# toandaominh1997/EfficientDet.Pytorch

Hardware: AMD Instinct MI355X
Metric: images/sec EfficientDet-D0 512px fwd+bwd (higher is better)
Workload: dtype f32_hf16x3_bwd_bf16x3

## Files before the change

efficientdet/pytorch_amd/_lib.py:

```python
import ctypes as C
import os

import torch

HERE = os.path.dirname(os.path.abspath(__file__))
LIB_PATH = os.environ.get('EFFDET_HIP_LIB') or os.path.join(os.path.dirname(os.path.abspath(__file__)), 'libeffdet_hip.so')
MAX_SEG = 5
MAX_CONV_SEG = 10
ABI_VERSION = 11
F32, BF16, F32_BF16X3, F32_SPLIT = 0, 1, 2, 3
F32_HSPLIT = 4
ACT_NONE, ACT_RELU, ACT_SWISH, ACT_SIGMOID = 0, 1, 2, 3
RES_NONE, RES_ADD, RES_RELU_MASK, RES_SWISH_GRAD = 0, 1, 2, 3
TUNE_IGEMM_BIG, TUNE_IGEMM_BIG_MIN_M, TUNE_SPLIT_PERS, TUNE_IGEMM_KORD, TUNE_SPLIT_KORD = 0, 1, 2, 3, 4

_ERR = {-1: 'EFFDET_EINVAL', -2: 'EFFDET_ELAUNCH', -3: 'EFFDET_EUNSUPPORTED'}


class Seg(C.Structure):
    _fields_ = [('H', C.c_int), ('W', C.c_int), ('Ho', C.c_int), ('Wo', C.c_int),
                ('in_off', C.c_longlong), ('in_bstride', C.c_longlong),
                ('out_off', C.c_longlong), ('out_bstride', C.c_longlong)]


# ... 195 lines not shown
}
SYMBOLS = list(SIGNATURES)
ADDED_SIGNATURES = {
    'effdet_soft_nms_workspace_bytes': 'q:iqi',
    'effdet_soft_nms': 'i:pppffifiiippppqiqs',
}
EMA_SIGNATURES = {
    'effdet_clip_adamw_step_ema': 'i:ppppppppiippffffffifipps',
    'effdet_clip_adamw_step_gated_ema': 'i:pppppppppiippfffffffippps',
    'effdet_ema_swap': 'i:pppppiis',
}
PLAN_SIGNATURES = {
    'effdet_dwconv_plan_info': 'i:iiiiiiiiiiiiip',
}
LIVE_SIGNATURES = {
    'effdet_live_tiles_counts': 'q:iipppp',
    'effdet_live_tiles': 'i:piiiippppps',
    'effdet_conv2d_live': 'i:ppis',
    'effdet_conv2d_wgrad_live': 'i:ppqps',
}
NEEDED_SIGNATURES = {
    'effdet_positive_pixel_map': 'i:ppiqiippps',
    'effdet_live_tiles_from_map': 'i:piippppps',
    'effdet_conv2d_needed': 'i:ppis',
}
BOX_LOSS_SIGNATURES = {
    'effdet_box_loss_fwd': 'i:ppppppqiqiiifs',
    'effdet_box_loss_fwd_grad': 'i:ppppppqpiiiqiiifs',
    'effdet_box_loss_bwd_reg': 'i:ppppppiiiqiifs',
}
LOSS_OPTS_SIGNATURES = {
    'effdet_loss_opts_workspace_bytes': 'q:iqii',
    'effdet_loss_opts_fwd': 'i:ppppppqiqiips',
    'effdet_loss_opts_fwd_grad': 'i:ppppppqpiiiqiips',
    'effdet_loss_opts_bwd_cls': 'i:pppppiiiqiips',
    'effdet_loss_opts_bwd_reg': 'i:ppppppiiiqips',
}
ATSS_SIGNATURES = {
    'effdet_loss_atss_workspace_bytes': 'q:iqiip',
    'effdet_loss_atss_fwd': 'i:ppppppqiqiipps',
    'effdet_loss_atss_fwd_grad': 'i:ppppppqpiiiqiipps',
}
CONV_PLAN_SIGNATURES = {
    'effdet_conv2d_plan_info': 'i:pp',
}
WBF_SIGNATURES = {
    'effdet_wbf_workspace_bytes': 'q:iii',
    'effdet_wbf': 'i:ppqs',
}
MOSAIC_SIGNATURES = {
    'effdet_mosaic_compose': 'i:ppppiiips',
    'effdet_mosaic_boxes': 'i:ppiipiffpips',
}
CONV_FORMS = ('plain', 'bf16x3', 'split', 'hsplit', 'skinny')
LIVE_RADII = 6
DW_PLAN_FWD, DW_PLAN_DGRAD, DW_PLAN_WGRAD, DW_PLAN_BWD, DW_PLAN_EXPAND_FWD = 0, 1, 2, 3, 4
DW_INFO = ('cq', 'tpi', 'ppt', 'nbuf', 'groups', 'nslab', 'direct')


def lib():
    global _lib
    if _lib is None:
        if not os.path.exists(LIB_PATH):
            raise RuntimeError(
                'libeffdet_hip.so is missing (%s). Build it with `python -m efficientdet.pytorch_amd.build` '
                '(or __graft_entry__.build()). There is no CPU fallback for this path.' % LIB_PATH)
        cand = C.CDLL(LIB_PATH)
        got = int(cand.effdet_abi_version()) if hasattr(cand, 'effdet_abi_version') else 0
        if got != ABI_VERSION:
            raise RuntimeError('%s has ABI generation %d, this binding needs %d: rebuild it (`python -m efficientdet.pytorch_amd.build`)'
                               % (LIB_PATH, got, ABI_VERSION))
        _lib = cand
        for name, sig in list(SIGNATURES.items()) + list(ADDED_SIGNATURES.items()) + list(EMA_SIGNATURES.items()) + \
                list(PLAN_SIGNATURES.items()) + list(LIVE_SIGNATURES.items()) + list(BOX_LOSS_SIGNATURES.items()) + \
                list(LOSS_OPTS_SIGNATURES.items()) + list(ATSS_SIGNATURES.items()) + list(CONV_PLAN_SIGNATURES.items()) + \
                list(WBF_SIGNATURES.items()) + list(NEEDED_SIGNATURES.items()) + list(MOSAIC_SIGNATURES.items()):
            f = getattr(_lib, name, None)
            if f is not None:
                f.restype, f.argtypes = _CTYPE[sig[0]], [_CTYPE[c] for c in sig[2:]]
    return _lib


def require(*names):
    L = lib()
    missing = [n for n in names if not hasattr(L, n)]
    if missing:
        raise RuntimeError('%s does not export %s: it predates this binding, rebuild it (`python -m efficientdet.pytorch_amd.build`)'
                           % (LIB_PATH, ', '.join(missing)))
    return L


def check(status, what):
    if status != 0:
        raise RuntimeError('%s failed: %s (%d)' % (what, _ERR.get(status, 'unknown'), status))


_raw_stream = getattr(torch._C, '_cuda_getCurrentRawStream', None)


def stream_ptr():
    if _raw_stream is not None:
        return _raw_stream(torch.cuda.current_device())
    return torch.cuda.current_stream().cuda_stream


def ptr(t):
    return None if t is None else t.data_ptr()


def dtype_code(t):
    if t == torch.float32:
        return F32
    if t == torch.bfloat16:
        return BF16
    raise TypeError('unsupported storage dtype %s' % t)
```

efficientdet/pytorch_amd/csrc/conv_wgrad.hip:

```cpp
#include "common.h"
#include "../../../include/effdet_live_tiles.h"
#include <stdlib.h>

#ifndef EFFDET_WGRAD_TR_WAVES
#define EFFDET_WGRAD_TR_WAVES 8
#endif

namespace {

struct WSeg {
  int H, W, Ho, Wo, M, split_start;
  long long in_off, in_bs, out_off, out_bs;
  unsigned x_bytes, dz_bytes;
  int step0;
};
struct WgradK {
  const void* x; const void* dz; float* dw; float* dbias; float* slab;
  float* dbp;
  int Cin, Cout, KW, stride, pad_t, pad_l;
  int ldx, lddz;
  int B;
  int Kc, cpt;
  int K;
  int mchunk;
  int nseg, ntiles, jtiles, vec_a;
  const unsigned char* live32;
  WSeg seg[EFFDET_MAX_SEG];
};

template <typename T> struct WMma;
template <> struct WMma<bf16_t> {
  static __device__ __forceinline__ void run(const uint4& a, const uint4& b, f32x4& c) {
    c = __builtin_amdgcn_mfma_f32_16x16x32_bf16(__builtin_bit_cast(bf16x8, a), __builtin_bit_cast(bf16x8, b), c, 0, 0, 0);
  }
  static __device__ __forceinline__ uint4 ones() { return make_uint4(0x3f803f80u, 0x3f803f80u, 0x3f803f80u, 0x3f803f80u); }
};
template <> struct WMma<float> {
  static __device__ __forceinline__ void run(const uint4& a, const uint4& b, f32x4& c) {
    c = __builtin_amdgcn_mfma_f32_16x16x4f32(__uint_as_float(a.x), __uint_as_float(b.x), c, 0, 0, 0);
    c = __builtin_amdgcn_mfma_f32_16x16x4f32(__uint_as_float(a.y), __uint_as_float(b.y), c, 0, 0, 0);
    c = __builtin_amdgcn_mfma_f32_16x16x4f32(__uint_as_float(a.z), __uint_as_float(b.z), c, 0, 0, 0);
    c = __builtin_amdgcn_mfma_f32_16x16x4f32(__uint_as_float(a.w), __uint_as_float(b.w), c, 0, 0, 0);
  }
  static __device__ __forceinline__ uint4 ones() { return make_uint4(0x3f800000u, 0x3f800000u, 0x3f800000u, 0x3f800000u); }
};

__device__ __forceinline__ int swz(int row) { return ((row >> 1) & 7) ^ ((row >> 4) & 7); }

template <typename T> struct Transpose;
template <> struct Transpose<float> {
  static __device__ __forceinline__ void run(const uint4 (&in)[4], uint4 (&out)[4]) {
    out[0] = make_uint4(in[0].x, in[1].x, in[2].x, in[3].x);
    out[1] = make_uint4(in[0].y, in[1].y, in[2].y, in[3].y);
    out[2] = make_uint4(in[0].z, in[1].z, in[2].z, in[3].z);
// ... 294 lines not shown
  }
  const bool want_bias = (p.dbp != nullptr) && (jt == 0) && (wj0 == 0);
  const uint4 ones = WMma<bf16_t>::ones();
  const int l15 = lane & 15, lq = lane >> 4;
  float* slab = p.slab + (long long)split * p.Cout * p.K;

  if (nsteps > 0) {
    stage(0);
    for (int kt = 0; kt < nsteps; ++kt) {
      const unsigned cur = (unsigned)(kt & 1) * BUFB;
      dma_wait_all();
      __syncthreads();
      if (kt + 1 < nsteps) stage((kt & 1) ^ 1);
#pragma unroll
      for (int ks = 0; ks < 2; ++ks) {
        uint4 af[4], bf[JT];
#pragma unroll
        for (int a = 0; a < 4; ++a) af[a] = frag(a_addr[a] + cur + (unsigned)ks * 8192u);
#pragma unroll
        for (int b = 0; b < JT; ++b) bf[b] = frag(b_addr[b] + cur + (unsigned)ks * 8192u);
#pragma unroll
        for (int a = 0; a < 4; ++a)
#pragma unroll
          for (int b = 0; b < JT; ++b) WMma<bf16_t>::run(af[a], bf[b], acc[a][b]);
        if (want_bias) {
#pragma unroll
          for (int a = 0; a < 4; ++a) WMma<bf16_t>::run(af[a], ones, bsum[a]);
        }
      }
    }
#pragma unroll
    for (int a = 0; a < 4; ++a) {
#pragma unroll
      for (int rr = 0; rr < 4; ++rr) {
        const int n = nt * 128 + wn0 + a * 16 + lq * 4 + rr;
        if (n >= p.Cout) continue;
#pragma unroll
        for (int b = 0; b < JT; ++b) {
          const int j = jt * 128 + wj0 + b * 16 + l15;
          if (j < p.K) slab[(long long)n * p.K + j] = acc[a][b][rr];
        }
        if (want_bias && l15 == 0) p.dbp[(long long)split * p.Cout + n] = bsum[a][rr];
      }
    }
  } else {
    for (int i = tid; i < 128 * 128; i += NW * 64) {
      const int n = nt * 128 + i / 128, j = jt * 128 + (i & 127);
      if (n < p.Cout && j < p.K) slab[(long long)n * p.K + j] = 0.f;
    }
    if (p.dbp && jt == 0 && tid < 128 && nt * 128 + tid < p.Cout) p.dbp[(long long)split * p.Cout + nt * 128 + tid] = 0.f;
  }
}

template <int ALLR, int LIVE = 0>
__global__ __launch_bounds__(512) void conv_wgrad_split_kernel(const WgradK p) {
  constexpr unsigned OPB = 16384, BUFB = 2 * OPB, RG = 4096;
  extern __shared__ __attribute__((aligned(16))) uint4 smem[];
  const int tid = threadIdx.x, lane = tid & 63;
  const int wave = __builtin_amdgcn_readfirstlane(tid >> 6);
  const int wn = wave >> 2, wj = wave & 3;
  const int logical = xcd_remap(blockIdx.x, gridDim.x);
  const int nt = logical % p.ntiles, jt = (logical / p.ntiles) % p.jtiles, split = logical / (p.ntiles * p.jtiles);
  int si = 0;
#pragma unroll
  for (int s = 1; s < EFFDET_MAX_SEG; ++s)
    if (s < p.nseg && split >= p.seg[s].split_start) si = s;
  const WSeg sg = p.seg[si];
  const int m_begin = (split - sg.split_start) * p.mchunk;
  const int m_end = min(sg.M, m_begin + p.mchunk);
  const int nsteps = (m_end - m_begin + 31) / 32;

  const bool stage_x = wave >= 4;
  const int rgi = wave & 3;
  const int Wr = sg.Wo < 8 ? sg.Wo : 8, RP = 8 / Wr;
  const int r = lane >> 3, g = (lane & 7) ^ (((r >> 1) & 3) << 1);
  const int dho = r / Wr, dwo = r - dho * Wr;
  int off_s[4]; unsigned flg[4];
#pragma unroll
  for (int hf = 0; hf < 4; ++hf) {
    if (!stage_x) {
      const int n = nt * 256 + hf * 64 + g * 8;
      off_s[hf] = (r * p.lddz + n) * 2;
      flg[hf] = (n + 8 > p.lddz) ? 1u : 0u;
    } else {
      const int jq = jt * 32 + hf * 8 + g;
      const bool jok = jq < p.Kc;
      const int tap = jok ? jq / p.cpt : 0, cc = jok ? jq - tap * p.cpt : 0;
      const int kh = tap / p.KW, kw = tap - kh * p.KW;
      const int dkh = kh - p.pad_t, dkw = kw - p.pad_l;
      off_s[hf] = ((dkh * sg.W + dkw + r) * p.ldx + cc * 8) * 2;
      flg[hf] = (jok ? 0u : 1u) | ((dkh < 0 && dho == 0) ? 2u : 0u) | ((dkh > 0 && dho == RP - 1) ? 4u : 0u) |
                ((dkw < 0 && dwo == 0) ? 8u : 0u) | ((dkw > 0 && dwo == Wr - 1) ? 16u : 0u);
    }
  }
  const u32x4_t srd = stage_x ? make_srd_raw((const bf16_t*)p.x + sg.in_off, sg.x_bytes)
                              : make_srd_raw((const bf16_t*)p.dz + sg.out_off, sg.dz_bytes);
  const u32x4_t srd_u = u32x4_t{(unsigned)__builtin_amdgcn_readfirstlane((int)srd[0]), (unsigned)__builtin_amdgcn_readfirstlane((int)srd[1]),
                                (unsigned)__builtin_amdgcn_readfirstlane((int)srd[2]), (unsigned)__builtin_amdgcn_readfirstlane((int)srd[3])};
  const unsigned s_bs = (unsigned)((stage_x ? sg.in_bs : sg.out_bs) * 2), s_ld = (unsigned)((stage_x ? p.ldx : p.lddz) * 2);
  const unsigned lds0 = lds_addr(smem);
  const unsigned dst0 = lds0 + (stage_x ? OPB : 0u) + (unsigned)rgi * RG;

  const int HoWo = sg.Ho * sg.Wo;
  int cm = m_begin + 8 * rgi;
  int cb = cm / HoWo, crem = cm - cb * HoWo;
  int cho = crem / sg.Wo, cwo = crem - cho * sg.Wo;
  auto seek = [&](int step) {
    cm = m_begin + 32 * step + 8 * rgi;
    cb = cm / HoWo; crem = cm - cb * HoWo;
    cho = crem / sg.Wo; cwo = crem - cho * sg.Wo;
  };
  const unsigned char* const lv = LIVE ? p.live32 + sg.step0 + m_begin / 32 : nullptr;
  int lwin = -1; unsigned long long lmask = 0ull;
  auto next_live = [&](int s) -> int {
    while (s < nsteps) {
      if ((s >> 6) != lwin) {
        lwin = s >> 6;
        const int i = lwin * 64 + lane;
        lmask = __ballot(i < nsteps && lv[i] != 0);
      }
      const unsigned long long rest = lmask >> (s & 63);
      if (rest) return s + __builtin_ctzll(rest);
      s = (s | 63) + 1;
    }
    return nsteps;
  };
  auto stage = [&](int buf) {
    const bool all_out = cm >= m_end;
    const unsigned cmask = 1u | (cho == 0 ? 2u : 0u) | (cho == sg.Ho - RP ? 4u : 0u) | (cwo == 0 ? 8u : 0u) | (cwo == sg.Wo - Wr ? 16u : 0u);
    const unsigned base = (unsigned)cb * s_bs + (unsigned)(cho * sg.Wo + cwo) * s_ld;
    const unsigned dst = dst0 + (unsigned)buf * BUFB;
#pragma unroll
    for (int hf = 0; hf < 4; ++hf)
      dma16_async(srd_u, dst + (unsigned)hf * 1024u, (all_out || (flg[hf] & cmask)) ? EFFDET_OOB : base + (unsigned)off_s[hf]);
    cm += 32; cwo += 32;
    while (cwo >= sg.Wo) { cwo -= sg.Wo; if (++cho == sg.Ho) { cho = 0; ++cb; } }
  };

  const int s16 = lane & 15, q = lane >> 4, jrow = s16 >> 2;
  const unsigned lane_base = (unsigned)(q >> 1) * RG + (unsigned)((q & 1) * 4 + jrow) * 128u + (unsigned)(s16 & 3) * 8u;
  const int xr = (q & 1) * 2 + (jrow >> 1);
  unsigned a_addr[2][4], b_addr[4];
#pragma unroll
  for (int gi = 0; gi < 2; ++gi)
#pragma unroll
    for (int k = 0; k < 4; ++k) a_addr[gi][k] = lds0 + lane_base + (unsigned)(2 * wn + gi) * 1024u + (unsigned)((k ^ xr) * 32);
#pragma unroll
  for (int k = 0; k < 4; ++k) b_addr[k] = lds0 + OPB + lane_base + (unsigned)wj * 1024u + (unsigned)((k ^ xr) * 32);
  auto frag = [&](unsigned addr) -> uint4 {
    const s16x4 lo = __builtin_amdgcn_ds_read_tr16_b64_v4i16((lds_s16x4_ptr)(size_t)addr);
    const s16x4 hi = __builtin_amdgcn_ds_read_tr16_b64_v4i16((lds_s16x4_ptr)(size_t)(addr + 2u * RG));
    const uint2 l2 = __builtin_bit_cast(uint2, lo), h2 = __builtin_bit_cast(uint2, hi);
    return make_uint4(l2.x, l2.y, h2.x, h2.y);
  };

  f32x4 acc[2][2][2], bsum[2][2];
#pragma unroll
  for (int gi = 0; gi < 2; ++gi)
#pragma unroll
    for (int a = 0; a < 2; ++a) {
      bsum[gi][a] = f32x4{0.f, 0.f, 0.f, 0.f};
#pragma unroll
      for (int b = 0; b < 2; ++b) acc[gi][a][b] = f32x4{0.f, 0.f, 0.f, 0.f};
    }
  const bool want_bias = (p.dbp != nullptr) && (jt == 0) && (wj == 0);
  const uint4 ones = WMma<bf16_t>::ones();
  const int l15 = lane & 15, lq = lane >> 4;
  float* slab = p.slab + (long long)split * p.Cout * p.K;
  const int n_alg0 = nt * 128 + wn * 64, j_alg0 = jt * 128 + wj * 32;

  int nxt = LIVE ? next_live(0) : 0;
  if (nxt < nsteps) {
    if constexpr (LIVE) { if (nxt != 0) seek(nxt); }
    stage(0);
    for (int kt = 0; LIVE ? nxt < nsteps : kt < nsteps; ++kt) {
      const unsigned cur = (unsigned)(kt & 1) * BUFB;
      dma_wait_all();
      __syncthreads();
      if constexpr (LIVE) {
        const int at = nxt + 1;
        nxt = next_live(at);
        if (nxt < nsteps) { if (nxt != at) seek(nxt); stage((kt & 1) ^ 1); }
      } else {
        if (kt + 1 < nsteps) stage((kt & 1) ^ 1);
      }
      uint4 bh[2], bl[2];
#pragma unroll
      for (int b = 0; b < 2; ++b) { bh[b] = frag(b_addr[b] + cur); bl[b] = frag(b_addr[2 + b] + cur); }
      if constexpr (ALLR) {
        uint4 ah[2][2], al[2][2];
#pragma unroll
        for (int gi = 0; gi < 2; ++gi)
#pragma unroll
          for (int a = 0; a < 2; ++a) { ah[gi][a] = frag(a_addr[gi][a] + cur); al[gi][a] = frag(a_addr[gi][2 + a] + cur); }
#pragma unroll
        for (int gi = 0; gi < 2; ++gi) {
#pragma unroll
          for (int t = 0; t < 3; ++t)
#pragma unroll
            for (int a = 0; a < 2; ++a)
#pragma unroll
              for (int b = 0; b < 2; ++b) WMma<bf16_t>::run(t == 0 ? al[gi][a] : ah[gi][a], t == 1 ? bl[b] : bh[b], acc[gi][a][b]);
          if (want_bias) {
#pragma unroll
            for (int a = 0; a < 2; ++a) { WMma<bf16_t>::run(al[gi][a], ones, bsum[gi][a]); WMma<bf16_t>::run(ah[gi][a], ones, bsum[gi][a]); }
          }
        }
      } else {
#pragma unroll
      for (int gi = 0; gi < 2; ++gi) {
        uint4 ah[2], al[2];
#pragma unroll
        for (int a = 0; a < 2; ++a) { ah[a] = frag(a_addr[gi][a] + cur); al[a] = frag(a_addr[gi][2 + a] + cur); }
#pragma unroll
        for (int t = 0; t < 3; ++t)
#pragma unroll
          for (int a = 0; a < 2; ++a)
#pragma unroll
            for (int b = 0; b < 2; ++b) WMma<bf16_t>::run(t == 0 ? al[a] : ah[a], t == 1 ? bl[b] : bh[b], acc[gi][a][b]);
        if (want_bias) {
#pragma unroll
          for (int a = 0; a < 2; ++a) { WMma<bf16_t>::run(al[a], ones, bsum[gi][a]); WMma<bf16_t>::run(ah[a], ones, bsum[gi][a]); }
        }
      }
      }
    }
#pragma unroll
    for (int gi = 0; gi < 2; ++gi)
#pragma unroll
      for (int a = 0; a < 2; ++a)
#pragma unroll
        for (int rr = 0; rr < 4; ++rr) {
          const int n = n_alg0 + gi * 32 + a * 16 + lq * 4 + rr;
          if (n >= p.Cout) continue;
#pragma unroll
          for (int b = 0; b < 2; ++b) {
            const int j = j_alg0 + b * 16 + l15;
            if (j < p.K) slab[(long long)n * p.K + j] = acc[gi][a][b][rr];
          }
          if (want_bias && l15 == 0) p.dbp[(long long)split * p.Cout + n] = bsum[gi][a][rr];
        }
  } else {
    for (int i = tid; i < 128 * 128; i += 512) {
      const int n = nt * 128 + i / 128, j = jt * 128 + (i & 127);
      if (n < p.Cout && j < p.K) slab[(long long)n * p.K + j] = 0.f;
    }
    if (p.dbp && jt == 0 && tid < 128 && nt * 128 + tid < p.Cout) p.dbp[(long long)split * p.Cout + nt * 128 + tid] = 0.f;
  }
}

template <int NW, int X3 = 0>
__global__ __launch_bounds__(NW * 64) void conv_wgrad_f32dma_kernel(const WgradK p) {
  constexpr int WJ = NW / 2;
  constexpr int WTJ = 128 / WJ, JB = WTJ / 16;
  constexpr int BKM = 32;
  constexpr unsigned OPB = 16384, BUFB = 2 * OPB;
  constexpr int PPW = 16 / NW;

  extern __shared__ __attribute__((aligned(16))) uint4 smem[];
  const int tid = threadIdx.x, lane = tid & 63;
  const int wave = __builtin_amdgcn_readfirstlane(tid >> 6);
  const int wn0 = (wave / WJ) * 64, wj0 = (wave % WJ) * WTJ;
  const int logical = xcd_remap(blockIdx.x, gridDim.x);
  const int nt = logical % p.ntiles, jt = (logical / p.ntiles) % p.jtiles, split = logical / (p.ntiles * p.jtiles);
  int si = 0;
#pragma unroll
  for (int s = 1; s < EFFDET_MAX_SEG; ++s)
    if (s < p.nseg && split >= p.seg[s].split_start) si = s;
  const WSeg sg = p.seg[si];
  const int m_begin = (split - sg.split_start) * p.mchunk;
  const int m_end = min(sg.M, m_begin + p.mchunk);
  const int nsteps = (m_end - m_begin + BKM - 1) / BKM;

  const int Wr = sg.Wo < 2 ? sg.Wo : 2, RP = 2 / Wr;
  const int r = lane >> 5, g = ((lane & 31) - 8 * r) & 31;
  const int dho = r / Wr, dwo = r - dho * Wr;
  const int n = nt * 128 + g * 4;
  const int off_z = (r * p.lddz + n) * 4;
  const unsigned long long mz_inv = __ballot(n + 4 > p.lddz);
  const int jq = jt * 32 + g;
  const bool jok = jq < p.Kc;
  const int tap = jok ? jq / p.cpt : 0, cc = jok ? jq - tap * p.cpt : 0;
  const int kh = tap / p.KW, kw = tap - kh * p.KW;
  const int dkh = kh - p.pad_t, dkw = kw - p.pad_l;
  const int off_x = (((dkh + dho * p.stride) * sg.W + dkw + dwo * p.stride) * p.ldx + cc * 4) * 4;
  const unsigned long long mx_inv = __ballot(!jok);
  const unsigned long long mx_up = __ballot(dkh < 0 && dho == 0), mx_dn = __ballot((sg.Ho - 1) * p.stride + dkh >= sg.H && dho == RP - 1);
  const unsigned long long mx_lf = __ballot(dkw < 0 && dwo == 0), mx_rt = __ballot((sg.Wo - 1) * p.stride + dkw >= sg.W && dwo == Wr - 1);
  const u32x4_t srd_x = make_srd_raw((const float*)p.x + sg.in_off, sg.x_bytes);
  const u32x4_t srd_z = make_srd_raw((const float*)p.dz + sg.out_off, sg.dz_bytes);
  const unsigned x_bs = (unsigned)(sg.in_bs * 4), x_ld = (unsigned)(p.ldx * 4), z_bs = (unsigned)(sg.out_bs * 4), z_ld = (unsigned)(p.lddz * 4);
  const unsigned lds0 = lds_addr(smem);
  const unsigned dst0 = lds0 + (unsigned)wave * 1024u;

  const int HoWo = sg.Ho * sg.Wo;
  int cm = m_begin + 2 * wave;
  int cb = cm / HoWo, crem = cm - cb * HoWo;
  int cho = crem / sg.Wo, cwo = crem - cho * sg.Wo;

  auto stage = [&](int buf) {
#pragma unroll
// ... 617 lines not shown
    k.live32 = live32;
    if (w.allr) {
      EFFDET_SET_MAX_LDS((conv_wgrad_split_kernel<1, 1>), w.lds);
      hipLaunchKernelGGL((conv_wgrad_split_kernel<1, 1>), dim3(tiles * w.splits), dim3(512), w.lds, st, k);
    } else {
      EFFDET_SET_MAX_LDS((conv_wgrad_split_kernel<0, 1>), w.lds);
      hipLaunchKernelGGL((conv_wgrad_split_kernel<0, 1>), dim3(tiles * w.splits), dim3(512), w.lds, st, k);
    }
  } else if (w.path == WG_SPLIT && w.allr) {
    EFFDET_SET_MAX_LDS(conv_wgrad_split_kernel<1>, w.lds);
    hipLaunchKernelGGL(conv_wgrad_split_kernel<1>, dim3(tiles * w.splits), dim3(512), w.lds, st, k);
  } else if (w.path == WG_SPLIT) {
    EFFDET_SET_MAX_LDS(conv_wgrad_split_kernel<0>, w.lds);
    hipLaunchKernelGGL(conv_wgrad_split_kernel<0>, dim3(tiles * w.splits), dim3(512), w.lds, st, k);
  } else if (w.path != WG_TILED) {
    w.thin(w, k, st);
  } else {
    WgradK ks = w.ks;
    ks.slab = k.slab + (long long)w.nfast * w.slab_floats;
    ks.dbp = k.dbp ? k.dbp + (long long)w.nfast * w.cout : nullptr;
    if (w.nfast > 0 && w.d.dtype == EFFDET_F32 && w.x3) {
      EFFDET_SET_MAX_LDS((conv_wgrad_f32dma_kernel<X3_NW, 1>), w.lds);
      hipLaunchKernelGGL((conv_wgrad_f32dma_kernel<X3_NW, 1>), dim3(tiles * w.nfast), dim3(X3_NW * 64), w.lds, st, k);
    } else if (w.nfast > 0 && w.d.dtype == EFFDET_F32) {
      EFFDET_SET_MAX_LDS((conv_wgrad_f32dma_kernel<F32_NW>), w.lds);
      hipLaunchKernelGGL(conv_wgrad_f32dma_kernel<F32_NW>, dim3(tiles * w.nfast), dim3(F32_NW * 64), w.lds, st, k);
    } else if (w.nfast > 0) {
      EFFDET_SET_MAX_LDS((conv_wgrad_tr_kernel<TR_NW>), w.lds);
      hipLaunchKernelGGL(conv_wgrad_tr_kernel<TR_NW>, dim3(tiles * w.nfast), dim3(TR_NW * 64), w.lds, st, k);
    }
    EFFDET_CHECK_LAUNCH();
    if (w.splits > w.nfast && w.d.dtype == EFFDET_F32) {
      EFFDET_SET_MAX_LDS((conv_wgrad_kernel<float>), w.lds);
      hipLaunchKernelGGL(conv_wgrad_kernel<float>, dim3(tiles * (w.splits - w.nfast)), dim3(256), w.lds, st, ks);
    } else if (w.splits > w.nfast) {
      EFFDET_SET_MAX_LDS((conv_wgrad_kernel<bf16_t>), w.lds);
      hipLaunchKernelGGL(conv_wgrad_kernel<bf16_t>, dim3(tiles * (w.splits - w.nfast)), dim3(256), w.lds, st, ks);
    }
  }
  EFFDET_CHECK_LAUNCH();
  return reduce_slabs(p, w, k.slab, k.dbp, st);
}

extern "C" int effdet_conv2d_wgrad(const effdet_wgrad_t* p, void* workspace, long long workspace_bytes,
                                   effdet_stream_t stream) {
  return wgrad_launch(p, workspace, workspace_bytes, nullptr, stream);
}

extern "C" int effdet_conv2d_wgrad_live(const effdet_wgrad_t* p, void* workspace, long long workspace_bytes,
                                        const unsigned char* live32, effdet_stream_t stream) {
  if (!live32) return EFFDET_EINVAL;
  return wgrad_launch(p, workspace, workspace_bytes, live32, stream);
}
```

efficientdet/pytorch_amd/functional.py:

```python
import os

import torch

from . import ops
from .config import BN_EPS, conv_out
from .ops import ACT_NONE, ACT_RELU, ACT_SIGMOID, ACT_SWISH, RES_ADD, RES_NONE, RES_RELU_MASK, Map

DW_SAVE_Y = os.environ.get('EFFDET_DW_SAVE_Y', '0') == '1'
BIFPN_WGRAD_GROUP = os.environ.get('EFFDET_BIFPN_WGRAD_GROUP', '1') != '0'
EXPAND_Z_ONLY = os.environ.get('EFFDET_EXPAND_Z_ONLY', '1') == '1'
SE_FUSED = os.environ.get('EFFDET_SE_FUSED', '1') == '1'
DW_BWD_FUSED = os.environ.get('EFFDET_DW_BWD_FUSED', '1') == '1'
PW_BWD_FUSED = os.environ.get('EFFDET_PW_BWD_FUSED', '1') == '1'
PW_DGRAD_SE = os.environ.get('EFFDET_PW_DGRAD_SE', '1') == '1'
FUSE_EXPAND_DW = os.environ.get('EFFDET_FUSE_EXPAND_DW', '1') == '1'
FUSE_CIN = tuple(int(v) for v in os.environ.get('EFFDET_FUSE_CIN', '16,24,32').split(','))
BIFPN_F16X3_MIN_WORK = float(os.environ.get('EFFDET_BIFPN_F16X3_MIN_WORK', '1.2e8'))
GATE_IN_WEIGHTS = os.environ.get('EFFDET_GATE_IN_WEIGHTS', '1') == '1'
GATE_IN_WEIGHTS_TRAIN = os.environ.get('EFFDET_GATE_IN_WEIGHTS_TRAIN', '0') == '1'


def chunk_elems(dtype):
    return 8 if dtype == torch.bfloat16 else 4

# ... 316 lines not shown


def level_tensor(m):
    n = m.B * m.H * m.W * m.C
    return m.t[m.off:m.off + n].view(m.B, m.H, m.W, m.C)


def head_out_maps(buf, B, sizes, per_anchor):
    A = sum(h * w for (h, w) in sizes) * 9
    maps, aoff = [], 0
    for (h, w) in sizes:
        maps.append(Map(buf, B, h, w, 9 * per_anchor, ld=9 * per_anchor, bstride=A * per_anchor, off=aoff * per_anchor))
        aoff += h * w * 9
    return maps


HEAD_TWO_STREAMS = os.environ.get('EFFDET_HEAD_TWO_STREAMS', '0') == '1'
_side_streams = {}


class _Fork:

    def __init__(self, device, on):
        self.on = on
        if on:
            key = (device.index, torch.cuda.current_stream(device).cuda_stream)
            if key not in _side_streams:
                _side_streams[key] = torch.cuda.Stream(device)
            self.main, self.s = torch.cuda.current_stream(device), _side_streams[key]

    def __enter__(self):
        if self.on:
            self.s.wait_stream(self.main)
        return self

    def side(self):
        import contextlib
        return torch.cuda.stream(self.s) if self.on else contextlib.nullcontext()

    def join(self):
        if self.on:
            self.main.wait_stream(self.s)
            self.on = False

    def __exit__(self, et, ev, tb):
        self.join()
        return False


HEAD_PAIR_TOWERS = os.environ.get('EFFDET_HEAD_PAIR_TOWERS', '1') == '1'
HEAD_SPLIT = os.environ.get('EFFDET_HEAD_SPLIT', '1') == '1'
HEAD_SPARSE_REG = os.environ.get('EFFDET_HEAD_SPARSE_REG', '1') == '1'
HEAD_SPARSE_REG_FWD = os.environ.get('EFFDET_HEAD_SPARSE_REG_FWD', '1') == '1'
_split_ok = {}


def head_uses_split(B, sizes, Wc, dtype, arith=None):
    if not (HEAD_SPLIT and dtype == torch.float32 and (arith or ops.F32_ARITH) == 'bf16x3' and Wc % 32 == 0):
        return False
    key = (B, tuple(sizes), Wc)
    if key not in _split_ok:
        _split_ok[key] = ops.wgrad_split_supported(B, sizes, 256, 256, 256) and ops.wgrad_split_supported(B, sizes, Wc, 256, 256)
    return _split_ok[key]


def _pyramid_to_split(src_maps, B, sizes, C_, dtype, dev, bf=True, h=False):
    dst = pyramid_alloc(B, sizes, C_, dtype, dev)[1] if bf else None
    dsth = pyramid_alloc(B, sizes, C_, dtype, dev)[1] if h else None
    for i, s_ in enumerate(src_maps):
        ops.to_split2(s_.tensor(), dst[i].addr() if bf else None, dsth[i].addr() if h else None, s_.B * s_.H * s_.W * s_.C,
                      ops.range_flag(dev) if h else None)
    return dst, dsth


def head_uses_f16x3(Wc, dtype):
    return HEAD_SPLIT and dtype == torch.float32 and ops.F32_ARITH == 'f32' and ops.F32_ARITH_HEAD == 'f16x3' and Wc % 32 == 0


def _head_forms(B, sizes, Wc, dtype, train):
    split = head_uses_split(B, sizes, Wc, dtype)
    split_bwd = (not split) and train and ops.F32_ARITH_BWD == 'bf16x3' and head_uses_split(B, sizes, Wc, dtype, 'bf16x3')
    hs = (not split) and head_uses_f16x3(Wc, dtype) and (split_bwd or not train)
    return split, split_bwd, hs


def head_fwd_takes_needed(p, dtype, train):
    _, split_bwd, hs = _head_forms(p[0].B, [(m.H, m.W) for m in p], p[0].C, dtype, train)
    return bool(HEAD_SPARSE_REG_FWD and train and hs and split_bwd)


def head_fwd(p, HP, num_classes, dtype, train, reg_needed=None):
    dev = p[0].t.device
    B, Wc = p[0].B, p[0].C
    sizes = [(m.H, m.W) for m in p]
    A = sum(h * w for (h, w) in sizes) * 9
    split, split_bwd, hs = _head_forms(B, sizes, Wc, dtype, train)
    if not (hs and split_bwd):
        reg_needed = None
    ntile = sum((B * h * w + 127) // 128 for (h, w) in sizes)

    def need(r):
        return reg_needed[r] if reg_needed is not None else None
    pin, pin_h = p, None
    if split or split_bwd or hs:
        pin, pin_h = _pyramid_to_split(p, B, sizes, Wc, dtype, dev, bf=split or split_bwd, h=hs)
        if pin is None:
# ... 61 lines not shown

def head_bwd(saved, dcls_logit, dreg, dtype, dcls_ld=0, cls_gscale=None, dreg_ld=0, in_split=False):
    p, acts, sizes, HP, nc, split = saved[:6]
    paired = len(saved) > 6 and saved[6] and split
    dev = p[0].t.device
    B, Wc = p[0].B, p[0].C
    g = {}
    apix = sum(h * w for (h, w) in sizes)
    last = {}
    live = None
    if HEAD_SPARSE_REG and split and dreg_ld and (in_split or dreg.dtype == torch.float32):
        live = ops.live_tiles(dreg, B, sizes, dreg_ld, in_split)
    ntile = sum((B * h * w + 127) // 128 for (h, w) in sizes)

    def lv(tower, kind, r):
        return live[kind][r] if (live is not None and tower == 'reg') else None

    def tower_final(tower, dout, per, pix_ld):
        fin = f'retina_{tower}'
        wf = HP[fin + '.weight']
        Cf = wf.shape[0]
        ce = 32 if split else chunk_elems(dtype)
        if pix_ld:
            Cfp, poff, dzmaps = pix_ld, 0, []
            for (h, w) in sizes:
                dzmaps.append(Map(dout, B, h, w, Cfp, ld=Cfp, bstride=apix * Cfp, off=poff * Cfp)); poff += h * w
            if split and not in_split:
                assert Cfp % 32 == 0
                dzmaps = _split_rows(dzmaps, Cfp, dtype)
        else:
            dzmaps = head_out_maps(dout, B, sizes, per)
            Cfp = (Cf + ce - 1) // ce * ce
            if split:
                dzmaps = _split_rows(dzmaps, Cfp, dtype)
            elif Cfp != Cf:
                dzmaps = [ops.pad_rows(m, Cfp) for m in dzmaps]
        G, dbp = ops.conv2d_wgrad(acts[tower][3], dzmaps, Cin=256, Cout=Cf, KH=3, KW=3, pad_t=1, pad_l=1, split=split, live32=lv(tower, 0, 0))
        gs = cls_gscale if tower == 'cls' else None
        dw = torch.empty_like(wf); db = ops.unpack_wgrad(G, dw, dbias_part=dbp, slab_scale=gs)
        rows = gs.expand(B).contiguous() if gs is not None else None
        g[fin + '.weight'], g[fin + '.bias'] = dw, db
        _, dz = pyramid_alloc(B, sizes, 256, dtype, dev)
        ops.conv2d(dzmaps, ops.pack_weight(wf, dtype, mode=1, cin_pad=Cfp, x3=split), dz, Cin=Cfp, Cout=256, KH=3, KW=3, pad_t=1,
                   pad_l=1, res=acts[tower][3], res_mode=RES_RELU_MASK, rowscale=rows, split=split, live=lv(tower, 1, 1))
        return dz

    def layer_wgrad(tower, t, dz):
        w = HP[f'{tower}_convs.{t}.weight']
        xin = acts[tower][t - 1] if t > 0 else p
        G, dbp = ops.conv2d_wgrad(xin, dz, Cin=w.shape[1], Cout=256, KH=3, KW=3, pad_t=1, pad_l=1, split=split, live32=lv(tower, 0, 4 - t))
        dw = torch.empty_like(w); db = ops.unpack_wgrad(G, dw, dbias_part=dbp)
        g[f'{tower}_convs.{t}.weight'], g[f'{tower}_convs.{t}.bias'] = dw, db

    def tower_bwd(tower, dout, per, pix_ld):
        dz = tower_final(tower, dout, per, pix_ld)
        for t in range(3, -1, -1):
            layer_wgrad(tower, t, dz)
            wd = ops.pack_weight(HP[f'{tower}_convs.{t}.weight'], dtype, mode=1, x3=split)
            if t > 0:
                _, nz = pyramid_alloc(B, sizes, 256, dtype, dev)
                ops.conv2d(dz, wd, nz, Cin=256, Cout=256, KH=3, KW=3, pad_t=1, pad_l=1, res=acts[tower][t - 1],
                           res_mode=RES_RELU_MASK, split=split, live=lv(tower, 1, 5 - t))
                dz = nz
            else:
                last[tower] = (dz, wd)

    if paired:
        dzs = {'reg': tower_final('reg', dreg, 4, dreg_ld), 'cls': tower_final('cls', dcls_logit, nc, dcls_ld)}
        L5 = len(sizes)
        for t in range(3, -1, -1):
            for tw in ('reg', 'cls'):
                layer_wgrad(tw, t, dzs[tw])
            wd2 = [ops.pack_weight(HP[f'{tw}_convs.{t}.weight'], dtype, mode=1, x3=split) for tw in ('cls', 'reg')]
            if t > 0:
                _, na, nb = pyramid_alloc_pair(B, sizes, 256, dtype, dev)
                ops.conv2d(dzs['cls'] + dzs['reg'], wd2[0], na + nb, Cin=256, Cout=256, KH=3, KW=3, pad_t=1, pad_l=1,
                           res=acts['cls'][t - 1] + acts['reg'][t - 1], res_mode=RES_RELU_MASK, split=split,
                           seg_w=[wd2[0]] * L5 + [wd2[1]] * L5, live=lv('reg', 1, 5 - t), live_tile0=ntile if live is not None else 0)
                dzs = {'cls': na, 'reg': nb}
            else:
                last['cls'], last['reg'] = (dzs['cls'], wd2[0]), (dzs['reg'], wd2[1])
    else:
        two = HEAD_TWO_STREAMS and ops.PROFILE is None
        ops.hold_tail_flush(two)
        try:
            with _Fork(dev, two) as fk:
                with fk.side():
                    tower_bwd('reg', dreg, 4, dreg_ld)
                tower_bwd('cls', dcls_logit, nc, dcls_ld)
        finally:
            ops.hold_tail_flush(False)
    _, dp_maps = pyramid_alloc(B, sizes, Wc, dtype, dev)
    dz, wd = last['cls']
    ops.conv2d(dz, wd, dp_maps, Cin=256, Cout=Wc, KH=3, KW=3, pad_t=1, pad_l=1, split=split, out_f32=split)
    dz, wd = last['reg']
    ops.conv2d(dz, wd, dp_maps, Cin=256, Cout=Wc, KH=3, KW=3, pad_t=1, pad_l=1, res=dp_maps, res_mode=RES_ADD, split=split, out_f32=split,
               live=lv('reg', 1, 5))
    return dp_maps, g
```

efficientdet/pytorch_amd/ops.py:

```python
import ctypes as C
import os
import threading

import numpy as np
import torch

from . import _lib as L
from ._lib import (ACT_NONE, ACT_RELU, ACT_SIGMOID, ACT_SWISH, RES_ADD, RES_NONE,
                   RES_RELU_MASK, RES_SWISH_GRAD)


class LaunchProfile:

    def __init__(self):
        self.records = []

    def summary(self):
        torch.cuda.synchronize()
        out = {}
        for name, flops, e0, e1, _, nbytes in self.records:
            d = out.setdefault(name, {'launches': 0, 'flops': 0.0, 'ms': 0.0, 'bytes': 0.0})
            d['launches'] += 1; d['flops'] += flops; d['ms'] += e0.elapsed_time(e1); d['bytes'] += nbytes
        return out

# ... 443 lines not shown
    d.B, d.Cin, d.Cout, d.KH, d.KW = x0.B, Cin, Cout, KH, KW
    d.stride, d.pad_t, d.pad_l = stride, pad_t, pad_l
    d.ldx, d.lddz = x0.ld, z0.ld
    d.image_splits = int(image_splits)
    _segs(d, xs, dzs, base_x, base_z, isz, z0.t.element_size())
    return d


def conv2d_wgrad_kernel_id(x, dz, *, Cin, Cout, KH, KW, stride=1, pad_t=0, pad_l=0, split=False):
    d = _wgrad_desc([x], [dz], None, None, Cin, Cout, KH, KW, stride, pad_t, pad_l, True, split, False)
    return int(L.lib().effdet_conv2d_wgrad_kernel(C.byref(d)))


def conv2d_wgrad(xs, dzs, dw=None, dbias=None, *, Cin, Cout, KH, KW, stride=1, pad_t=0, pad_l=0, want_bias=True, split=False,
                 image_splits=False, group=False, live32=None):
    if isinstance(xs, Map):
        xs, dzs = [xs], [dzs]
    x0 = xs[0]
    d = _wgrad_desc(xs, dzs, dw, dbias, Cin, Cout, KH, KW, stride, pad_t, pad_l, want_bias, split, image_splits)
    flops = 2.0 * KH * KW * Cin * Cout * sum(z.B * z.H * z.W for z in dzs)
    splits = int(L.lib().effdet_conv2d_wgrad_splits(C.byref(d)))
    if splits < 1:
        raise RuntimeError('effdet_conv2d_wgrad: unsupported geometry')
    n = Cout * KH * KW * Cin
    ws = torch.empty(splits * (n + Cout), dtype=torch.float32, device=x0.t.device)
    nbytes = ws.numel() * 4
    if live32 is not None:
        assert split and live32.dtype == torch.uint8 and live32.is_contiguous()
        assert live32.numel() == sum((z.B * z.H * z.W + 31) // 32 for z in dzs)
        run = lambda: L.check(L.require('effdet_conv2d_wgrad_live').effdet_conv2d_wgrad_live(C.byref(d), L.ptr(ws), nbytes, live32.data_ptr(),
                                                                                             L.stream_ptr()), 'effdet_conv2d_wgrad_live')
    else:
        run = lambda: L.check(L.lib().effdet_conv2d_wgrad(C.byref(d), L.ptr(ws), nbytes, L.stream_ptr()), 'effdet_conv2d_wgrad')
    _timed('conv_wgrad_tr_kernel<8>' if x0.dtype == torch.bfloat16 else
           ('conv_wgrad_split_kernel' if split else
            ('conv_wgrad_thin_kernel' if int(L.lib().effdet_conv2d_wgrad_kernel(C.byref(d))) == 1 else
             ('conv_wgrad_f32dma_kernel<4,bf16x3>' if d.dtype == L.F32_BF16X3 else 'conv_wgrad_f32dma_kernel<8>'))), flops,
           run,
           'k%d s%d Cin%d Cout%d M%d' % (KH, stride, Cin, Cout, sum(z.B * z.H * z.W for z in dzs)),
           nbytes=float(x0.t.element_size() * Cin * sum(x.B * x.H * x.W for x in xs) +
                        dzs[0].t.element_size() * Cout * sum(z.B * z.H * z.W for z in dzs) + 4.0 * splits * (n + Cout)))
    slabs = ws[:splits * n].view(splits, Cout, KH * KW, Cin)
    parts = ws[splits * n:].view(splits, Cout) if d.dbias else None
    if group:
        assert dw is None and not image_splits
        first, count = (C.c_int * len(xs))(), (C.c_int * len(xs))()
        tot = int(L.lib().effdet_conv2d_wgrad_seg_slabs(C.byref(d), first, count))
        assert tot == splits
        return [(slabs[first[i]:first[i] + count[i]], parts[first[i]:first[i] + count[i]] if parts is not None else None)
                for i in range(len(xs))]
    return slabs, parts


class _TailBatch:

    def __init__(self):
        self.jobs, self.keep, self.bytes = [], [], 0

    def add(self, kind, job, *tensors):
        t = L.TailJob()
        t.kind = kind
        if kind == L.TAIL_UNPACK:
            t.u.conv = job
        elif kind == L.TAIL_SE_PARAMS:
            t.u.se = job
        else:
            t.u.dw = job
        self.jobs.append(t); self.keep.append(tensors)
        self.bytes += sum(x.numel() * x.element_size() for x in tensors if isinstance(x, torch.Tensor))
        if self.bytes > TAIL_KEEP_BYTES and not getattr(_tls, 'hold_tail', False):
            self.flush()

    def flush(self):
        if self.jobs:
            arr = (L.TailJob * len(self.jobs))(*self.jobs)
            L.check(L.lib().effdet_backward_tail(arr, len(self.jobs), L.stream_ptr()), 'effdet_backward_tail')
        self.jobs, self.keep, self.bytes = [], [], 0


UNPACK_BATCHED = os.environ.get('EFFDET_UNPACK_BATCH', '1') != '0'
TAIL_KEEP_BYTES = int(os.environ.get('EFFDET_TAIL_KEEP_MB', '2048')) << 20


def hold_tail_flush(on):
    _tls.hold_tail = bool(on)


def _cur_batch():
    return getattr(_tls, 'unpack_batch', None)


class unpack_batch:

    def __enter__(self):
        self.owner = _cur_batch() is None and UNPACK_BATCHED
        if self.owner:
            _tls.unpack_batch = _TailBatch()
        return self

    def __exit__(self, et, ev, tb):
        if self.owner:
            b, _tls.unpack_batch = _tls.unpack_batch, None
            if et is None:
                b.flush()
        return False

# ... 1265 lines not shown
```

Measured before the change: 1342.

## Fuse cls and reg head tower weight-gradient convs into one paired launch

Adds a paired wgrad kernel that runs the cls and reg tower weight-gradient split GEMMs for the same layer in a single grid. Blocks are distributed per XCD between the two problems, and the sparse reg problem (live mask) is scheduled with a different split/tile order. The goal is to cut launch count and to fill the GPU better than two back-to-back smaller launches, particularly when the reg side is sparse. It adds a new C entry point, a Python wrapper and an env toggle, enabled by default. Each problem still needs its own slab reduction.

```diff
diff --git a/efficientdet/pytorch_amd/_lib.py b/efficientdet/pytorch_amd/_lib.py
--- a/efficientdet/pytorch_amd/_lib.py
+++ b/efficientdet/pytorch_amd/_lib.py
@@ -271,6 +271,9 @@
     'effdet_mosaic_compose': 'i:ppppiiips',
     'effdet_mosaic_boxes': 'i:ppiipiffpips',
 }
+WGRAD_PAIR_SIGNATURES = {
+    'effdet_conv2d_wgrad_pair': 'i:pppqps',
+}
 CONV_FORMS = ('plain', 'bf16x3', 'split', 'hsplit', 'skinny')
 LIVE_RADII = 6
 DW_PLAN_FWD, DW_PLAN_DGRAD, DW_PLAN_WGRAD, DW_PLAN_BWD, DW_PLAN_EXPAND_FWD = 0, 1, 2, 3, 4
@@ -293,7 +296,8 @@
         for name, sig in list(SIGNATURES.items()) + list(ADDED_SIGNATURES.items()) + list(EMA_SIGNATURES.items()) + \
                 list(PLAN_SIGNATURES.items()) + list(LIVE_SIGNATURES.items()) + list(BOX_LOSS_SIGNATURES.items()) + \
                 list(LOSS_OPTS_SIGNATURES.items()) + list(ATSS_SIGNATURES.items()) + list(CONV_PLAN_SIGNATURES.items()) + \
-                list(WBF_SIGNATURES.items()) + list(NEEDED_SIGNATURES.items()) + list(MOSAIC_SIGNATURES.items()):
+                list(WBF_SIGNATURES.items()) + list(NEEDED_SIGNATURES.items()) + list(MOSAIC_SIGNATURES.items()) + \
+                list(WGRAD_PAIR_SIGNATURES.items()):
             f = getattr(_lib, name, None)
             if f is not None:
                 f.restype, f.argtypes = _CTYPE[sig[0]], [_CTYPE[c] for c in sig[2:]]
diff --git a/efficientdet/pytorch_amd/csrc/conv_wgrad.hip b/efficientdet/pytorch_amd/csrc/conv_wgrad.hip
--- a/efficientdet/pytorch_amd/csrc/conv_wgrad.hip
+++ b/efficientdet/pytorch_amd/csrc/conv_wgrad.hip
@@ -1,5 +1,6 @@
 #include "common.h"
 #include "../../../include/effdet_live_tiles.h"
+#include "../../../include/effdet_wgrad_pair.h"
 #include <stdlib.h>
 
 #ifndef EFFDET_WGRAD_TR_WAVES
@@ -400,20 +401,14 @@
   }
 }
 
-template <int ALLR, int LIVE = 0>
-__global__ __launch_bounds__(512) void conv_wgrad_split_kernel(const WgradK p) {
+template <int ALLR, int LIVE>
+__device__ __forceinline__ void wgrad_split_block(const WgradK& p, const WSeg& sg, const void* const px, const void* const pdz, float* const pslab,
+                                                  float* const pdbp, const unsigned char* const plive, const int nt, const int jt, const int split) {
   constexpr unsigned OPB = 16384, BUFB = 2 * OPB, RG = 4096;
   extern __shared__ __attribute__((aligned(16))) uint4 smem[];
   const int tid = threadIdx.x, lane = tid & 63;
   const int wave = __builtin_amdgcn_readfirstlane(tid >> 6);
   const int wn = wave >> 2, wj = wave & 3;
-  const int logical = xcd_remap(blockIdx.x, gridDim.x);
-  const int nt = logical % p.ntiles, jt = (logical / p.ntiles) % p.jtiles, split = logical / (p.ntiles * p.jtiles);
-  int si = 0;
-#pragma unroll
-  for (int s = 1; s < EFFDET_MAX_SEG; ++s)
-    if (s < p.nseg && split >= p.seg[s].split_start) si = s;
-  const WSeg sg = p.seg[si];
   const int m_begin = (split - sg.split_start) * p.mchunk;
   const int m_end = min(sg.M, m_begin + p.mchunk);
   const int nsteps = (m_end - m_begin + 31) / 32;
@@ -441,8 +436,8 @@
                 ((dkw < 0 && dwo == 0) ? 8u : 0u) | ((dkw > 0 && dwo == Wr - 1) ? 16u : 0u);
     }
   }
-  const u32x4_t srd = stage_x ? make_srd_raw((const bf16_t*)p.x + sg.in_off, sg.x_bytes)
-                              : make_srd_raw((const bf16_t*)p.dz + sg.out_off, sg.dz_bytes);
+  const u32x4_t srd = stage_x ? make_srd_raw((const bf16_t*)px + sg.in_off, sg.x_bytes)
+                              : make_srd_raw((const bf16_t*)pdz + sg.out_off, sg.dz_bytes);
   const u32x4_t srd_u = u32x4_t{(unsigned)__builtin_amdgcn_readfirstlane((int)srd[0]), (unsigned)__builtin_amdgcn_readfirstlane((int)srd[1]),
                                 (unsigned)__builtin_amdgcn_readfirstlane((int)srd[2]), (unsigned)__builtin_amdgcn_readfirstlane((int)srd[3])};
   const unsigned s_bs = (unsigned)((stage_x ? sg.in_bs : sg.out_bs) * 2), s_ld = (unsigned)((stage_x ? p.ldx : p.lddz) * 2);
@@ -458,7 +453,7 @@
     cb = cm / HoWo; crem = cm - cb * HoWo;
     cho = crem / sg.Wo; cwo = crem - cho * sg.Wo;
   };
-  const unsigned char* const lv = LIVE ? p.live32 + sg.step0 + m_begin / 32 : nullptr;
+  const unsigned char* const lv = LIVE ? plive + sg.step0 + m_begin / 32 : nullptr;
   int lwin = -1; unsigned long long lmask = 0ull;
   auto next_live = [&](int s) -> int {
     while (s < nsteps) {
@@ -511,10 +506,10 @@
 #pragma unroll
       for (int b = 0; b < 2; ++b) acc[gi][a][b] = f32x4{0.f, 0.f, 0.f, 0.f};
     }
-  const bool want_bias = (p.dbp != nullptr) && (jt == 0) && (wj == 0);
+  const bool want_bias = (pdbp != nullptr) && (jt == 0) && (wj == 0);
   const uint4 ones = WMma<bf16_t>::ones();
   const int l15 = lane & 15, lq = lane >> 4;
-  float* slab = p.slab + (long long)split * p.Cout * p.K;
+  float* slab = pslab + (long long)split * p.Cout * p.K;
   const int n_alg0 = nt * 128 + wn * 64, j_alg0 = jt * 128 + wj * 32;
 
   int nxt = LIVE ? next_live(0) : 0;
@@ -586,15 +581,58 @@
             const int j = j_alg0 + b * 16 + l15;
             if (j < p.K) slab[(long long)n * p.K + j] = acc[gi][a][b][rr];
           }
-          if (want_bias && l15 == 0) p.dbp[(long long)split * p.Cout + n] = bsum[gi][a][rr];
+          if (want_bias && l15 == 0) pdbp[(long long)split * p.Cout + n] = bsum[gi][a][rr];
         }
   } else {
     for (int i = tid; i < 128 * 128; i += 512) {
       const int n = nt * 128 + i / 128, j = jt * 128 + (i & 127);
       if (n < p.Cout && j < p.K) slab[(long long)n * p.K + j] = 0.f;
     }
-    if (p.dbp && jt == 0 && tid < 128 && nt * 128 + tid < p.Cout) p.dbp[(long long)split * p.Cout + nt * 128 + tid] = 0.f;
-  }
+    if (pdbp && jt == 0 && tid < 128 && nt * 128 + tid < p.Cout) pdbp[(long long)split * p.Cout + nt * 128 + tid] = 0.f;
+  }
+}
+
+
+template <int ALLR, int LIVE = 0>
+__global__ __launch_bounds__(512) void conv_wgrad_split_kernel(const WgradK p) {
+  const int logical = xcd_remap(blockIdx.x, gridDim.x);
+  const int nt = logical % p.ntiles, jt = (logical / p.ntiles) % p.jtiles, split = logical / (p.ntiles * p.jtiles);
+  int si = 0;
+#pragma unroll
+  for (int s = 1; s < EFFDET_MAX_SEG; ++s)
+    if (s < p.nseg && split >= p.seg[s].split_start) si = s;
+  wgrad_split_block<ALLR, LIVE>(p, p.seg[si], p.x, p.dz, p.slab, p.dbp, p.live32, nt, jt, split);
+}
+
+struct WgradPairK {
+  WgradK k;
+  const void* x[2]; const void* dz[2];
+  float* slab[2]; float* dbp[2];
+  const unsigned char* live32;
+  int nseg[2], splits[2];
+  int first;
+  WSeg seg[2][EFFDET_MAX_SEG];
+};
+
+template <int ALLR, int LIVEB>
+__global__ __launch_bounds__(512) void conv_wgrad_pair_kernel(const WgradPairK q) {
+  const int tiles = q.k.ntiles * q.k.jtiles;
+  const int xcd = (int)blockIdx.x & 7, idx = (int)blockIdx.x >> 3;
+  auto eighth = [](int n, int x) { return x * (n >> 3) + min(x, n & 7); };
+  const int f0 = eighth(tiles * q.splits[q.first], xcd), nf = eighth(tiles * q.splits[q.first], xcd + 1) - f0;
+  const int prob = idx < nf ? q.first : q.first ^ 1;
+  const int l = idx < nf ? f0 + idx : eighth((int)gridDim.x, xcd) - f0 + (idx - nf);
+  int split, tile;
+  if (LIVEB && prob == 1) { tile = l / q.splits[1]; split = q.splits[1] - 1 - (l - tile * q.splits[1]); }
+  else { split = l / tiles; tile = l - split * tiles; }
+  const int nt = tile % q.k.ntiles, jt = tile / q.k.ntiles;
+  int si = 0;
+#pragma unroll
+  for (int s = 1; s < EFFDET_MAX_SEG; ++s)
+    if (s < q.nseg[prob] && split >= q.seg[prob][s].split_start) si = s;
+  const WSeg sg = q.seg[prob][si];
+  if (LIVEB && prob == 1) wgrad_split_block<ALLR, 1>(q.k, sg, q.x[1], q.dz[1], q.slab[1], q.dbp[1], q.live32, nt, jt, split);
+  else wgrad_split_block<ALLR, 0>(q.k, sg, q.x[prob], q.dz[prob], q.slab[prob], q.dbp[prob], nullptr, nt, jt, split);
 }
 
 template <int NW, int X3 = 0>
@@ -1318,3 +1356,55 @@
   if (!live32) return EFFDET_EINVAL;
   return wgrad_launch(p, workspace, workspace_bytes, live32, stream);
 }
+
+extern "C" int effdet_conv2d_wgrad_pair(const effdet_wgrad_t* a, const effdet_wgrad_t* b, void* workspace, long long workspace_bytes,
+                                        const unsigned char* live32_b, effdet_stream_t stream) {
+  if (!a || !b || !a->x || !a->dz || !b->x || !b->dz || !workspace) return EFFDET_EINVAL;
+  WgradPlan wa, wb;
+  int rc = plan_wgrad(a, wa);
+  if (rc != EFFDET_OK) return rc;
+  rc = plan_wgrad(b, wb);
+  if (rc != EFFDET_OK) return rc;
+  if (wa.path != WG_SPLIT || wb.path != WG_SPLIT) return EFFDET_EUNSUPPORTED;
+  const WgradK &ka = wa.k, &kb = wb.k;
+  if (ka.Cin != kb.Cin || ka.Cout != kb.Cout || a->KH != b->KH || a->KW != b->KW || ka.stride != kb.stride || ka.pad_t != kb.pad_t ||
+      ka.pad_l != kb.pad_l || ka.ldx != kb.ldx || ka.lddz != kb.lddz || ka.B != kb.B || ka.mchunk != kb.mchunk || wa.allr != wb.allr ||
+      ka.ntiles != kb.ntiles || ka.jtiles != kb.jtiles || ka.K != kb.K || ka.Kc != kb.Kc || ka.cpt != kb.cpt || wa.lds != wb.lds)
+    return EFFDET_EUNSUPPORTED;
+  if (workspace_bytes < wa.workspace_bytes + wb.workspace_bytes) return EFFDET_EINVAL;
+  if (live32_b && ka.mchunk % 32) return EFFDET_EINVAL;
+  hipStream_t st = (hipStream_t)stream;
+  WgradPairK q;
+  q.k = ka;
+  const WgradPlan* w[2] = {&wa, &wb};
+  const effdet_wgrad_t* d[2] = {a, b};
+  float* base = (float*)workspace;
+  for (int i = 0; i < 2; ++i) {
+    q.x[i] = w[i]->k.x; q.dz[i] = w[i]->k.dz;
+    q.slab[i] = base;
+    q.dbp[i] = d[i]->dbias ? base + (long long)w[i]->splits * w[i]->slab_floats : nullptr;
+    q.nseg[i] = w[i]->k.nseg; q.splits[i] = w[i]->splits;
+    for (int s = 0; s < EFFDET_MAX_SEG; ++s) q.seg[i][s] = w[i]->k.seg[s];
+    base += w[i]->workspace_bytes / (long long)sizeof(float);
+  }
+  q.live32 = live32_b;
+  const char* ord = getenv("EFFDET_WGRAD_PAIR_ORDER");
+  q.first = ord ? (atoi(ord) ? 1 : 0) : (live32_b ? 1 : 0);
+  const unsigned grid = (unsigned)(ka.ntiles * ka.jtiles) * (unsigned)(wa.splits + wb.splits);
+  if (live32_b && wa.allr) {
+    EFFDET_SET_MAX_LDS((conv_wgrad_pair_kernel<1, 1>), wa.lds);
+    hipLaunchKernelGGL((conv_wgrad_pair_kernel<1, 1>), dim3(grid), dim3(512), wa.lds, st, q);
+  } else if (live32_b) {
+    EFFDET_SET_MAX_LDS((conv_wgrad_pair_kernel<0, 1>), wa.lds);
+    hipLaunchKernelGGL((conv_wgrad_pair_kernel<0, 1>), dim3(grid), dim3(512), wa.lds, st, q);
+  } else if (wa.allr) {
+    EFFDET_SET_MAX_LDS((conv_wgrad_pair_kernel<1, 0>), wa.lds);
+    hipLaunchKernelGGL((conv_wgrad_pair_kernel<1, 0>), dim3(grid), dim3(512), wa.lds, st, q);
+  } else {
+    EFFDET_SET_MAX_LDS((conv_wgrad_pair_kernel<0, 0>), wa.lds);
+    hipLaunchKernelGGL((conv_wgrad_pair_kernel<0, 0>), dim3(grid), dim3(512), wa.lds, st, q);
+  }
+  EFFDET_CHECK_LAUNCH();
+  rc = reduce_slabs(a, wa, q.slab[0], q.dbp[0], st);
+  return rc != EFFDET_OK ? rc : reduce_slabs(b, wb, q.slab[1], q.dbp[1], st);
+}
diff --git a/efficientdet/pytorch_amd/functional.py b/efficientdet/pytorch_amd/functional.py
--- a/efficientdet/pytorch_amd/functional.py
+++ b/efficientdet/pytorch_amd/functional.py
@@ -392,6 +392,7 @@
 HEAD_SPLIT = os.environ.get('EFFDET_HEAD_SPLIT', '1') == '1'
 HEAD_SPARSE_REG = os.environ.get('EFFDET_HEAD_SPARSE_REG', '1') == '1'
 HEAD_SPARSE_REG_FWD = os.environ.get('EFFDET_HEAD_SPARSE_REG_FWD', '1') == '1'
+HEAD_PAIR_WGRAD = os.environ.get('EFFDET_HEAD_PAIR_WGRAD', '1') == '1'
 _split_ok = {}
 
 
@@ -559,6 +560,15 @@
         dw = torch.empty_like(w); db = ops.unpack_wgrad(G, dw, dbias_part=dbp)
         g[f'{tower}_convs.{t}.weight'], g[f'{tower}_convs.{t}.bias'] = dw, db
 
+    def layer_wgrad_pair(t, dz_cls, dz_reg):
+        ws = [HP[f'{tw}_convs.{t}.weight'] for tw in ('cls', 'reg')]
+        xin = [acts[tw][t - 1] if t > 0 else p for tw in ('cls', 'reg')]
+        res = ops.conv2d_wgrad_pair(xin[0], dz_cls, xin[1], dz_reg, Cin=ws[0].shape[1], Cout=256, KH=3, KW=3, pad_t=1, pad_l=1,
+                                    live32_b=lv('reg', 0, 4 - t))
+        for tw, w, (G, dbp) in reversed(list(zip(('cls', 'reg'), ws, res))):
+            dw = torch.empty_like(w); db = ops.unpack_wgrad(G, dw, dbias_part=dbp)
+            g[f'{tw}_convs.{t}.weight'], g[f'{tw}_convs.{t}.bias'] = dw, db
+
     def tower_bwd(tower, dout, per, pix_ld):
         dz = tower_final(tower, dout, per, pix_ld)
         for t in range(3, -1, -1):
@@ -576,8 +586,11 @@
         dzs = {'reg': tower_final('reg', dreg, 4, dreg_ld), 'cls': tower_final('cls', dcls_logit, nc, dcls_ld)}
         L5 = len(sizes)
         for t in range(3, -1, -1):
-            for tw in ('reg', 'cls'):
-                layer_wgrad(tw, t, dzs[tw])
+            if HEAD_PAIR_WGRAD:
+                layer_wgrad_pair(t, dzs['cls'], dzs['reg'])
+            else:
+                for tw in ('reg', 'cls'):
+                    layer_wgrad(tw, t, dzs[tw])
             wd2 = [ops.pack_weight(HP[f'{tw}_convs.{t}.weight'], dtype, mode=1, x3=split) for tw in ('cls', 'reg')]
             if t > 0:
                 _, na, nb = pyramid_alloc_pair(B, sizes, 256, dtype, dev)
diff --git a/efficientdet/pytorch_amd/ops.py b/efficientdet/pytorch_amd/ops.py
--- a/efficientdet/pytorch_amd/ops.py
+++ b/efficientdet/pytorch_amd/ops.py
@@ -519,6 +519,37 @@
     return slabs, parts
 
 
+def conv2d_wgrad_pair(xs_a, dzs_a, xs_b, dzs_b, *, Cin, Cout, KH, KW, stride=1, pad_t=0, pad_l=0, want_bias=True, live32_b=None):
+    if isinstance(xs_a, Map):
+        xs_a, dzs_a = [xs_a], [dzs_a]
+    if isinstance(xs_b, Map):
+        xs_b, dzs_b = [xs_b], [dzs_b]
+    lib_ = L.require('effdet_conv2d_wgrad_pair')
+    ds = [_wgrad_desc(xs, dzs, None, None, Cin, Cout, KH, KW, stride, pad_t, pad_l, want_bias, True, False)
+          for xs, dzs in ((xs_a, dzs_a), (xs_b, dzs_b))]
+    splits = [int(lib_.effdet_conv2d_wgrad_splits(C.byref(d))) for d in ds]
+    if min(splits) < 1:
+        raise RuntimeError('effdet_conv2d_wgrad_pair: unsupported geometry')
+    n = Cout * KH * KW * Cin
+    ws = torch.empty(sum(splits) * (n + Cout), dtype=torch.float32, device=xs_a[0].t.device)
+    nbytes = ws.numel() * 4
+    if live32_b is not None:
+        assert live32_b.dtype == torch.uint8 and live32_b.is_contiguous()
+        assert live32_b.numel() == sum((z.B * z.H * z.W + 31) // 32 for z in dzs_b)
+    run = lambda: L.check(lib_.effdet_conv2d_wgrad_pair(C.byref(ds[0]), C.byref(ds[1]), L.ptr(ws), nbytes, L.ptr(live32_b), L.stream_ptr()),
+                          'effdet_conv2d_wgrad_pair')
+    pix = sum(z.B * z.H * z.W for z in dzs_a) + sum(z.B * z.H * z.W for z in dzs_b)
+    _timed('conv_wgrad_split_kernel', 2.0 * KH * KW * Cin * Cout * pix, run, 'pair k%d s%d Cin%d Cout%d M%d' % (KH, stride, Cin, Cout, pix),
+           nbytes=float(xs_a[0].t.element_size() * Cin * (sum(x.B * x.H * x.W for x in xs_a) + sum(x.B * x.H * x.W for x in xs_b)) +
+                        dzs_a[0].t.element_size() * Cout * pix + 4.0 * sum(splits) * (n + Cout)))
+    out, o = [], 0
+    for sp in splits:
+        slabs = ws[o:o + sp * n].view(sp, Cout, KH * KW, Cin)
+        parts = ws[o + sp * n:o + sp * (n + Cout)].view(sp, Cout) if want_bias else None
+        out.append((slabs, parts)); o += sp * (n + Cout)
+    return tuple(out)
+
+
 class _TailBatch:
 
     def __init__(self):
diff --git a/include/effdet_wgrad_pair.h b/include/effdet_wgrad_pair.h
--- /dev/null
+++ b/include/effdet_wgrad_pair.h
@@ -0,0 +1,14 @@
+#ifndef EFFDET_WGRAD_PAIR_H
+#define EFFDET_WGRAD_PAIR_H
+#include "effdet_hip.h"
+#ifdef __cplusplus
+extern "C" {
+#endif
+
+int effdet_conv2d_wgrad_pair(const effdet_wgrad_t* a, const effdet_wgrad_t* b, void* workspace, long long workspace_bytes,
+                             const unsigned char* live32_b, effdet_stream_t stream);
+
+#ifdef __cplusplus
+}
+#endif
+#endif
```

After: 1366 (median of 6 runs). 1.8% higher.
